# MasterVVK/qwen3-tts-axera-russian

Hardware: AMD Instinct MI355X
Metric: 12Hz codec-tokens/s (codec frames/s, 16 codes each) + RTF, Qwen3-TTS-0.6B (higher is better)
Workload: dtype f16 weights/KV, f32 accumulate (talker+CP); vocoder exact fp32 (f32 MFMA); 1 GPU; configs[2]/[3]: batch=32 mixed ru/en prompts per GPU, 64 frames/utterance/step (prefill + hipGraph decode loop), utterance-sharded DP over 1 GPU(s); batch_per_gpu=32

## Files before the change

### qwen3_tts_axera_russian_amd/csrc/q3_kernels.h

```cpp
#pragma once
#include "q3_common.h"
#include "q3_frag.h"

namespace q3 {

enum { PRO_F16 = 0, PRO_NORM = 1 };
enum { EPI_STORE = 0, EPI_RESID = 1, EPI_SWIGLU = 2 };

struct LinArgs {
    int tl_node = -1;
    const half_t* wp = nullptr;
    int N = 0, K = 0, M = 0;
    int m_begin = 0;
    int swap_grid = 0;
    int nt = 0;
    const half_t* x16 = nullptr;
    const float* ssq = nullptr;
    int ssq_parts = 0;
    float eps = 1e-6f;
    float* y = nullptr;
    int ldy = 0;
    float* h_out = nullptr;
    float* ssq_out = nullptr;
    half_t* xh_out = nullptr;
    const float* gamma = nullptr;
    half_t* act = nullptr;
};
int launch_linear(hipStream_t s, const LinArgs& a, int pro, int epi);
int linear_decode_kbw(int K, int N, int rows);

int launch_pack_linear(hipStream_t s, const half_t* src, int N, int K, half_t* dst, int tile_off,
                       int tile_stride);

enum { ATTN_FUSED = 0, ATTN_PREP = 1, ATTN_ATTEND = 2 };
struct AttnArgs {
    int tl_node = -1;
    float* qkv = nullptr;
// ... 163 lines not shown
    int seen_vocab = 0;
    const float* talker_emb = nullptr;
    int talker_vocab = 0;
    const float* const* cp_tables = nullptr;
    int cp_vocab = 0, n_groups = 15;
    const float* pad_embed = nullptr;
    float* h = nullptr;
    float* ssq = nullptr;
    half_t* xh = nullptr;
    const float* gamma = nullptr;
    int row0 = 0, max_rows = 0, H = 0;
};
int launch_prompt_rows(hipStream_t s, const PromptRowsArgs& a);

int tl_next_node();

int set_linear_tuning(int K, int mt16, int kbw);
int set_linear_split_rows(int on);
int set_linear_narrow8(int on);
int set_linear_wide_tiles(int on);
int set_attn_short(int on);
int set_gemm_min_rows(int n);
int set_gemm_glds(int on);
int reset_linear_knobs();
const char* last_linear_variant();

}
```

### qwen3_tts_axera_russian_amd/csrc/q3_linear.hip

```cpp
#include "q3_kdev.h"

namespace q3 {

__global__ void pack_linear_kernel(const half_t* __restrict__ src, int N, int K, half_t* __restrict__ dst,
                                   int tile_off, int tile_stride) {
    const int KB = K / 32;
    size_t idx = (size_t)blockIdx.x * blockDim.x + threadIdx.x;
    size_t total = (size_t)(N / 16) * KB * 64;
    if (idx >= total) return;
    int lane = (int)(idx & 63);
    size_t blk = idx >> 6;
    int kb = (int)(blk % KB);
    int ts = (int)(blk / KB);
    int n = ts * 16 + (lane & 15);
    int k = kb * 32 + (lane >> 4) * 8;
    h8 v = *(const h8*)(src + (size_t)n * K + k);
    size_t td = (size_t)tile_off + (size_t)ts * tile_stride;
    *(h8*)(dst + ((td * KB + kb) * 64 + lane) * 8) = v;
}

int launch_pack_linear(hipStream_t s, const half_t* src, int N, int K, half_t* dst, int tile_off,
                       int tile_stride) {
    if (N % 16 || K % 32) {
        Q3_LOG("pack_linear: N=%d K=%d not multiples of 16/32", N, K);
// ... 195 lines not shown
    const unsigned nt_ = a.N / (16 * NB16), nr_ = (a.M - a.m_begin + MR - 1) / MR;
    b.swap_grid = nr_ > 2 ? 1 : 0;
    dim3 grid(b.swap_grid ? nr_ : nt_, b.swap_grid ? nt_ : nr_);
    const void* asrc = (const void*)b.x16;
    void* outp = EPI == EPI_STORE ? (void*)b.y : EPI == EPI_RESID ? (void*)b.h_out : (void*)b.act;
    hipLaunchKernelGGL((linear_kernel<NB16, MT16, KBW, NW, PRO, EPI, NT>), grid, dim3(NW * 64), lds, s, b.wp, asrc, b.ssq,
                       b.gamma, outp, b.M, b.N, b.m_begin, b.swap_grid, b.eps, b);
    Q3_HIP(hipGetLastError(), -1);
    return 0;
}

__device__ __forceinline__ void gemm_tile_of_block(int R, int T, int& row_tile, int& col_tile) {
    const int L = blockIdx.x;
    if (T % 8 == 0) {
        const int x = L & 7, j = L >> 3;
        row_tile = j % R;
        col_tile = x + 8 * (j / R);
    } else {
        row_tile = L % R;
        col_tile = L / R;
    }
}

template <int BM, int BN, int PRO, int EPI>
__device__ __forceinline__ void gemm_epilogue(const LinArgs& a, f4 (&acc)[BM / 32][BN / 32], const float* post, int m0,
                                              int tile0, int wm, int wn, int q, int c) {
    constexpr int WM = BM / 32, WN = BN / 32;
#pragma unroll
    for (int i = 0; i < WM; i++) {
#pragma unroll
        for (int r = 0; r < 4; r++) {
            const int mr = (wm * WM + i) * 16 + 4 * q + r;
            const int m = m0 + mr;
            const bool ok = m < a.M;
            const float ps = PRO == PRO_NORM ? post[mr] : 1.0f;
            if (EPI == EPI_SWIGLU) {
#pragma unroll
                for (int j = 0; j < WN; j += 2) {
                    const float g = acc[i][j][r] * ps, u = acc[i][j + 1][r] * ps;
                    const float sg = __fdividef(g, 1.0f + __expf(-g));
                    const int jn = ((tile0 + wn * WN + j) >> 1) * 16 + c;
                    if (ok) a.act[frag_idx(m, jn, a.N / 2)] = sat_half(sg * u);
                }
            } else {
#pragma unroll
                for (int j = 0; j < WN; j++) {
                    const int ng = (tile0 + wn * WN + j) * 16 + c;
                    const float v = acc[i][j][r] * ps;
                    if (EPI == EPI_STORE) {
                        if (ok) a.y[(size_t)m * a.ldy + ng] = v;
                    } else {
                        const size_t hi = frag_idx(m, ng, a.N);
                        const float hn = ok ? a.h_out[hi] + v : 0.f;
                        if (ok) a.h_out[hi] = hn;
                        if (ok && a.xh_out) a.xh_out[hi] = pre_scaled(hn, a.gamma[ng]);
                        const float s2 = group_sum_down<16>(hn * hn);
                        if (ok && c == 0) a.ssq_out[(size_t)m * (a.N / 16) + (ng >> 4)] = s2;
                    }
                }
            }
        }
    }
}

template <int BM, int BN, int KS, int PRO, int EPI>
__global__ void __launch_bounds__(256) gemm_kernel(LinArgs a) {
    constexpr int RA = BM / 16, RB = BN / 16;
    constexpr int NF = (RA + RB) * KS, FPW = NF / 4;
    constexpr int WM = BM / 32, WN = BN / 32;
    static_assert(NF % 4 == 0 && WN % 2 == 0, "tile shape");
    Q3_TL(20 + PRO * 4 + EPI);
    const int tid = threadIdx.x, lane = tid & 63, w = tid >> 6;
    const int wm = w >> 1, wn = w & 1, q = lane >> 4, c = lane & 15;
    int row_tile, col_tile;
    gemm_tile_of_block((a.M - a.m_begin + BM - 1) / BM, a.N / BN, row_tile, col_tile);
    const int m0 = a.m_begin + row_tile * BM;
    const int tile0 = col_tile * RB;
    const int KB = a.K >> 5, NST = KB / KS;
// ... 42 lines not shown
            for (int i = 0; i < FPW; i++) st[i] = *frag_ptr(w * FPW + i, (ks + 1) * KS);
        }
        const h8* cur = lds + (size_t)(ks & 1) * NF * 64;
#pragma unroll
        for (int kk = 0; kk < KS; kk++) {
            h8 af[WM], bf[WN];
#pragma unroll
            for (int i = 0; i < WM; i++) af[i] = cur[((wm * WM + i) * KS + kk) * 64 + lane];
#pragma unroll
            for (int j = 0; j < WN; j++) bf[j] = cur[(RA * KS + (wn * WN + j) * KS + kk) * 64 + lane];
#pragma unroll
            for (int i = 0; i < WM; i++)
#pragma unroll
                for (int j = 0; j < WN; j++)
                    acc[i][j] = __builtin_amdgcn_mfma_f32_16x16x32_f16(af[i], bf[j], acc[i][j], 0, 0, 0);
        }
        if (more) {
            h8* nxt = lds + (size_t)((ks + 1) & 1) * NF * 64;
#pragma unroll
            for (int i = 0; i < FPW; i++) nxt[(w * FPW + i) * 64 + lane] = st[i];
        }
        __syncthreads();
    }
    gemm_epilogue<BM, BN, PRO, EPI>(a, acc, post, m0, tile0, wm, wn, q, c);
}

template <int N>
__device__ __forceinline__ void wait_vmcnt() {
    asm volatile("s_waitcnt vmcnt(%0)" ::"n"(N) : "memory");
}

template <int BM, int BN, int NBUF, int PRO, int EPI, int KS = 2>
__global__ void __launch_bounds__(512) gemm_glds_kernel(LinArgs a) {
    constexpr int RA = BM / 16, RB = BN / 16;
    static_assert(KS % 2 == 0, "two wave groups share a stage's k-blocks");
    constexpr int NF = (RA + RB) * KS, FPW = NF / 8;
    constexpr int WM = BM / 32, WN = BN / 32;
    constexpr int PF = NBUF - 1;
    static_assert(NF % 8 == 0 && WN % 2 == 0, "tile shape");
    static_assert((size_t)NBUF * NF * 1024 >= (size_t)4 * WM * WN * 4 * 64 * 4, "the ring must hold one group's accumulators");
    Q3_TL(24 + PRO * 4 + EPI);
    const int tid = threadIdx.x, lane = tid & 63, w = tid >> 6;
    const int grp = w >> 2, wq = w & 3;
    const int wm = wq >> 1, wn = wq & 1, q = lane >> 4, c = lane & 15;
    int row_tile, col_tile;
    gemm_tile_of_block((a.M - a.m_begin + BM - 1) / BM, a.N / BN, row_tile, col_tile);
    const int m0 = a.m_begin + row_tile * BM;
// ... 25 lines not shown
        for (int r = tid; r < BM; r += 512) {
            const int m = m0 + r;
            float sum = 0.f;
            if (m < a.M) {
                const float4* sp = (const float4*)(a.ssq + (size_t)m * 64);
#pragma unroll
                for (int p = 0; p < 16; p++) {
                    const float4 v = sp[p];
                    sum += (v.x + v.y) + (v.z + v.w);
                }
            }
            post[r] = (1.0f / sqrtf(sum / (float)a.K + a.eps)) * NORM_POST;
        }
    }
    asm volatile("s_waitcnt vmcnt(0)" ::: "memory");
#pragma unroll
    for (int st = 0; st < PF; st++)
        if (st < NST) issue(st);
    f4 acc[WM][WN];
#pragma unroll
    for (int i = 0; i < WM; i++)
#pragma unroll
        for (int j = 0; j < WN; j++) acc[i][j] = (f4){0.f, 0.f, 0.f, 0.f};
    for (int ks = 0; ks < NST; ks++) {
        const int ahead = NST - 1 - ks;
        if (ahead >= PF - 1) wait_vmcnt<(PF - 1) * FPW>();
        else if (PF > 2 && ahead == 1) wait_vmcnt<FPW>();
        else wait_vmcnt<0>();
        __builtin_amdgcn_s_barrier();
        asm volatile("" ::: "memory");
        if (ks + PF < NST) issue(ks + PF);
        const h8* cur = lds + (size_t)(ks % NBUF) * NF * 64;
#pragma unroll
        for (int kk = 0; kk < KS / 2; kk++) {
            const int kb = grp * (KS / 2) + kk;
            h8 af[WM], bf[WN];
#pragma unroll
            for (int i = 0; i < WM; i++) af[i] = cur[((wm * WM + i) * KS + kb) * 64 + lane];
#pragma unroll
            for (int j = 0; j < WN; j++) bf[j] = cur[(RA * KS + (wn * WN + j) * KS + kb) * 64 + lane];
#pragma unroll
            for (int i = 0; i < WM; i++)
#pragma unroll
                for (int j = 0; j < WN; j++)
                    acc[i][j] = __builtin_amdgcn_mfma_f32_16x16x32_f16(af[i], bf[j], acc[i][j], 0, 0, 0);
        }
    }
    __builtin_amdgcn_s_barrier();
    asm volatile("" ::: "memory");
    f4* xch = (f4*)smem;
    if (grp == 1) {
#pragma unroll
        for (int i = 0; i < WM; i++)
#pragma unroll
            for (int j = 0; j < WN; j++) xch[((size_t)wq * WM * WN + i * WN + j) * 64 + lane] = acc[i][j];
    }
    __syncthreads();
    if (grp == 1) return;
#pragma unroll
    for (int i = 0; i < WM; i++)
#pragma unroll
        for (int j = 0; j < WN; j++) {
            const f4 o = xch[((size_t)wq * WM * WN + i * WN + j) * 64 + lane];
            acc[i][j] += o;
        }
    gemm_epilogue<BM, BN, PRO, EPI>(a, acc, post, m0, tile0, wm, wn, q, c);
}

static int g_gemm_glds = env_int("Q3_GEMM_GLDS", 1);
int set_gemm_glds(int on) { g_gemm_glds = on; return 0; }

template <int BM, int BN, int PRO, int EPI>
static int launch_gemm_t(hipStream_t s, const LinArgs& a) {
    LinArgs b = a;
    b.tl_node = tl_next_node();
    dim3 grid(((a.M - a.m_begin + BM - 1) / BM) * (a.N / BN));
    if (g_gemm_glds) {
#ifndef Q3_GEMM_KS_SMALL
#define Q3_GEMM_KS_SMALL 4
#endif
        constexpr int NBUF = (BM + BN) > 256 ? 3 : 4;
        constexpr int KS2 = (BM + BN) <= 128 ? Q3_GEMM_KS_SMALL : 2;
        constexpr size_t lds2 = (size_t)NBUF * ((BM + BN) / 16) * KS2 * 1024 + BM * 4;
        static bool attr2 = false;
        if (!attr2) {
            Q3_HIP(hipFuncSetAttribute((const void*)gemm_glds_kernel<BM, BN, NBUF, PRO, EPI, KS2>,
                                       hipFuncAttributeMaxDynamicSharedMemorySize, (int)lds2), -1);
            attr2 = true;
        }
        if ((a.K >> 5) % KS2) {
            Q3_LOG("launch_gemm: K=%d is no multiple of %d", a.K, 32 * KS2);
            return -1;
        }
        static char name[64];
        if (!name[0])
            snprintf(name, sizeof(name), "gemm_glds<%d,%d,%d,%s,%s,%d>", BM, BN, NBUF, pro_name(PRO), epi_name(EPI), KS2);
        g_last_variant = name;
        hipLaunchKernelGGL((gemm_glds_kernel<BM, BN, NBUF, PRO, EPI, KS2>), grid, dim3(512), lds2, s, b);
    } else if constexpr (BM + BN <= 256) {
        constexpr int KS = 1024 / (BM + BN);
        constexpr size_t lds = (size_t)2 * ((BM + BN) / 16) * KS * 1024;
        static bool attr_set = false;
        if (!attr_set) {
            if (lds > 48 * 1024)
                Q3_HIP(hipFuncSetAttribute((const void*)gemm_kernel<BM, BN, KS, PRO, EPI>,
                                           hipFuncAttributeMaxDynamicSharedMemorySize, (int)lds), -1);
            attr_set = true;
        }
        static char name[64];
        if (!name[0]) snprintf(name, sizeof(name), "gemm<%d,%d,%d,%s,%s>", BM, BN, KS, pro_name(PRO), epi_name(EPI));
        g_last_variant = name;
        hipLaunchKernelGGL((gemm_kernel<BM, BN, KS, PRO, EPI>), grid, dim3(256), lds, s, b);
    } else {
        Q3_LOG("launch_gemm: no register-staged %d x %d tile", BM, BN);
        return -1;
    }
    Q3_HIP(hipGetLastError(), -1);
    return 0;
}
// ... 115 lines not shown
    else
        hipLaunchKernelGGL((linear_narrow_kernel<KBW, NW, false>), dim3(64, groups), dim3(NW * 64), 0, s, a.wp, a.x16, a.h_out, a.gamma,
                           a.ssq_out, a.xh_out, a.M, a.m_begin, node);
    Q3_HIP(hipGetLastError(), -1);
    return 0;
}

#define Q3_LIN_CASE(NB16_, MT16_, KBW_, NW_, PRO_, EPI_)                                   \
    if (nb16 == NB16_ && mt16 == MT16_ && kbw == KBW_ && nw == NW_ && pro == PRO_ && epi == EPI_) \
        return launch_linear_t<NB16_, MT16_, KBW_, NW_, PRO_, EPI_>(s, a);

#define Q3_LIN_MT(NB16_, KBW_, NW_, PRO_, EPI_) \
    Q3_LIN_CASE(NB16_, 1, KBW_, NW_, PRO_, EPI_) \
    Q3_LIN_CASE(NB16_, 2, KBW_, NW_, PRO_, EPI_) \
    Q3_LIN_CASE(NB16_, 4, KBW_, NW_, PRO_, EPI_)

int reset_linear_knobs() {
    memcpy(g_tune_kbw, g_tune_kbw_default, sizeof(g_tune_kbw));
    g_wide_tiles = 0;
    g_split_rows_narrow = 1;
    g_gemm_min_rows = 65;
    g_narrow8 = env_int("Q3_LINEAR_NARROW8", 1);
    g_gemm_glds = env_int("Q3_GEMM_GLDS", 1);
    return 0;
}

static int decode_mt16(int rows, int N) {
    int mt16 = rows <= 16 ? 1 : rows <= 32 ? 2 : 4;
    if (rows > 16 && rows <= 32 && ((g_split_rows_narrow == 1 && N <= 1024) || g_split_rows_narrow == 2)) mt16 = 1;
    return mt16;
}

int linear_decode_kbw(int K, int N, int rows) {
    const int ki = K == 1024 ? 0 : K == 2048 ? 1 : K == 3072 ? 2 : -1;
    if (rows <= 0 || rows >= g_gemm_min_rows || ki < 0 || N % 32) return 0;
    const int mt16 = decode_mt16(rows, N);
    return g_tune_kbw[ki][mt16 == 1 ? 0 : mt16 == 2 ? 1 : 2];
}

int launch_linear(hipStream_t s, const LinArgs& a, int pro, int epi) {
    g_last_variant = "";
    const int rows = a.M - a.m_begin;
    if (rows <= 0) return 0;
    if (rows >= g_gemm_min_rows) return launch_gemm(s, a, pro, epi);
    const int K = a.K;
    int ki = K == 1024 ? 0 : K == 2048 ? 1 : K == 3072 ? 2 : -1;
// ... 32 lines not shown
```

### qwen3_tts_axera_russian_amd/csrc/q3_sample.hip

```cpp
#include "q3_kdev.h"

namespace q3 {

__device__ __forceinline__ void block_argmax(float& v, int& idx, float* sv, int* si) {
    group_argmax_down<64>(v, idx);
    const int w = threadIdx.x >> 6, nw = blockDim.x >> 6;
    if ((threadIdx.x & 63) == 0) {
        sv[w] = v;
        si[w] = idx;
    }
    __syncthreads();
    v = sv[0];
    idx = si[0];
    for (int i = 1; i < nw; i++)
        if (sv[i] > v || (sv[i] == v && si[i] < idx)) {
            v = sv[i];
            idx = si[i];
        }
    __syncthreads();
}

__device__ __forceinline__ float uniform01(unsigned long long seed, unsigned row, unsigned frame, unsigned group) {
    unsigned long long z = seed + 0x9E3779B97F4A7C15ull * (1ull + row + ((unsigned long long)frame << 20) +
                                                            ((unsigned long long)group << 44));
// ... 148 lines not shown
        }
        chosen = pick;
    }
    __syncthreads();
    return chosen;
}

template <class T>
__device__ __forceinline__ T uniform_entry(const T* p, int r) {
    static_assert(sizeof(T) % 4 == 0, "the entry is read as words");
    constexpr int NW = (int)(sizeof(T) / 4);
    const __attribute__((address_space(4))) int* q = (const __attribute__((address_space(4))) int*)(p + r);
    int w[NW];
#pragma unroll
    for (int i = 0; i < NW; i++) w[i] = q[i];
    T e;
    __builtin_memcpy(&e, w, sizeof(e));
    return e;
}
__device__ __forceinline__ SlotParams uniform_slot(const SlotParams* p, int r) { return uniform_entry(p, r); }
__device__ __forceinline__ SlotRules uniform_rules(const SlotRules* p, int r) { return uniform_entry(p, r); }

template <bool SLOTS, bool RULES = false, bool SCORES = false>
__device__ __forceinline__ void talker_sample_row(const TalkerSampleArgs& a) {
    Q3_TL(42);
    __shared__ float sv[16];
    __shared__ int si[16];
    __shared__ float sc_wm[SCORES ? 16 : 1], sc_ws[SCORES ? 16 : 1];
    float sc_m = -INFINITY, sc_s = 0.f;
    __shared__ int win[32];
    __shared__ int nwin;
    const int r = a.row0 + blockIdx.x;
    const int RT = a.R_total > 0 ? a.R_total : a.R;
    const int np = uniform_load(a.n_past + r);
    const int nt = uniform_load(a.n_text + r);
    const bool was_done = uniform_load(a.done + r) != 0;
    float temperature = a.temperature, top_p = a.top_p;
    int top_k = a.top_k, max_frames = a.max_frames;
    int slot_flags = 0;
    if constexpr (SLOTS) {
        const SlotParams sp = uniform_slot(a.slots, r);
        temperature = sp.t_temp;
        top_p = sp.t_top_p;
        top_k = sp.t_top_k;
        max_frames = sp.max_frames;
        slot_flags = sp.flags;
        if (a.text_avail) {
// ... 117 lines not shown
        } else {
            fc[0] = code;
            if constexpr (SCORES) {
                if (a.scores) {
                    const int nw = blockDim.x >> 6;
                    float m = sc_wm[0], sum = 0.f;
                    for (int i = 1; i < nw; i++) m = fmaxf(m, sc_wm[i]);
                    for (int i = 0; i < nw; i++) sum += sc_wm[i] > -INFINITY ? sc_ws[i] * expf(sc_wm[i] - m) : 0.f;
                    float zu = -INFINITY;
                    if (used >= 0 && used < a.V && (used < a.audio_vocab || used == a.eos))
                        zu = nan_as_inf(a.logits[(size_t)r * a.V + used]);
                    a.scores[((size_t)f * RT + r) * 16] = (m < INFINITY && m > -INFINITY) ? zu - m - logf(sum) : __builtin_nanf("");
                }
            }
            a.past[r * 32 + (np & 31)] = used;
            if constexpr (RULES)
                if (a.seen && used >= 0 && used < a.audio_vocab)
                    a.seen[(size_t)r * ((a.audio_vocab + 31) / 32) + (used >> 5)] |= 1u << (used & 31);
            a.n_past[r] = np + 1;
            a.pos[r] = a.pos0[r] + np;
        }
    }
}
__global__ void talker_sample_kernel(TalkerSampleArgs a) { talker_sample_row<false>(a); }
__global__ void talker_sample_kernel_slots(TalkerSampleArgs a) { talker_sample_row<true>(a); }
__global__ void talker_sample_kernel_rules(TalkerSampleArgs a) { talker_sample_row<true, true>(a); }
__global__ void talker_sample_kernel_scores(TalkerSampleArgs a) { talker_sample_row<false, false, true>(a); }
__global__ void talker_sample_kernel_slots_scores(TalkerSampleArgs a) { talker_sample_row<true, false, true>(a); }
__global__ void talker_sample_kernel_rules_scores(TalkerSampleArgs a) { talker_sample_row<true, true, true>(a); }

static size_t sample_lds_bytes_slots(int n) { return (size_t)sample_sort_len(n) * 8; }

static int sample_vocab_refused(const char* who, bool slots, int V, float temperature, int top_k) {
    if (slots && V > SAMPLE_SORT_CAP) {
        Q3_LOG("%s: a vocabulary of %d is beyond the per-slot sampler (sort cap %d)", who, V, SAMPLE_SORT_CAP);
        return -1;
    }
    if (temperature > 1e-6f && effective_top_k(top_k, V) > SAMPLE_SEL_CAP && V > SAMPLE_SORT_CAP) {
        Q3_LOG("%s: top_k=%d over a vocabulary of %d is beyond the device sampler (sort cap %d)", who, top_k, V, SAMPLE_SORT_CAP);
        return -1;
    }
    return 0;
}

int launch_talker_sample(hipStream_t s, const TalkerSampleArgs& a) {
    if (a.R <= 0) return 0;
    if ((a.text_avail && !a.held) || ((a.text_avail || a.held) && !a.slots)) {
        Q3_LOG("talker_sample: text_avail / held need each other and per-slot mode (text_avail %p, held %p, slots %p)",
               (const void*)a.text_avail, (const void*)a.held, (const void*)a.slots);
        return -1;
    }
    if ((a.rules || a.seen) && (!a.slots || (a.rules && !a.seen) || a.audio_vocab <= 0)) {
        Q3_LOG("talker_sample: rules need seen, and both per-slot mode (rules %p, seen %p, slots %p)", (const void*)a.rules,
               (const void*)a.seen, (const void*)a.slots);
        return -1;
    }
    if (sample_vocab_refused("talker_sample", a.slots != nullptr, a.V, a.temperature, a.top_k)) return -1;
    const size_t lds = a.slots ? sample_lds_bytes_slots(a.V) : sample_lds_bytes(a.V, a.top_k, a.temperature);
    TalkerSampleArgs a2 = a;
    a2.tl_node = tl_next_node();
    static void (*const kernels[2][3])(TalkerSampleArgs) = {
        {talker_sample_kernel, talker_sample_kernel_slots, talker_sample_kernel_rules},
        {talker_sample_kernel_scores, talker_sample_kernel_slots_scores, talker_sample_kernel_rules_scores}};
    hipLaunchKernelGGL(kernels[a.scores ? 1 : 0][(a.rules || a.seen) ? 2 : a.slots ? 1 : 0], dim3(a.R), dim3(256), lds, s, a2);
    Q3_HIP(hipGetLastError(), -1);
    return 0;
}

template <bool SLOTS, bool RULES = false, bool SCORES = false>
__device__ __forceinline__ void cp_argmax_row(const CpArgmaxArgs& a) {
    if constexpr (SLOTS)
        Q3_FETCH_ARGS("s"(a.logits), "s"(a.V), "s"(a.H), "s"(a.row0), "s"(a.R_total), "s"(a.R), "s"(a.group), "s"(a.codes), "s"(a.n_frames),
                      "s"(a.frame_cap), "s"(a.next_table), "s"(a.h_out), "s"(a.ssq_out), "s"(a.xh_out), "s"(a.gamma_next),
                      "s"(a.talker_emb), "s"(a.slots), "s"(a.forced), "s"(a.next_qkv), "s"(a.qkv_out), "s"(a.qkv_ld),
                      "s"(a.text_rows), "s"(a.text_avail), "s"(a.text_cap), "s"(a.held));
    else
        Q3_FETCH_ARGS("s"(a.logits), "s"(a.V), "s"(a.H), "s"(a.row0), "s"(a.R_total), "s"(a.R), "s"(a.group), "s"(a.codes), "s"(a.n_frames),
                      "s"(a.frame_cap), "s"(a.next_table), "s"(a.h_out), "s"(a.ssq_out), "s"(a.xh_out), "s"(a.gamma_next),
                      "s"(a.talker_emb), "s"(a.temperature), "s"(a.forced), "s"(a.next_qkv), "s"(a.qkv_out), "s"(a.qkv_ld));
    Q3_TL(43);
    __shared__ float sv[4];
    __shared__ int si[4];
    const int r = a.row0 + blockIdx.x, tid = threadIdx.x;
    const int RT = a.R_total > 0 ? a.R_total : a.R;
    float best = -INFINITY;
    int bidx = 0x7fffffff;
    const float4* lg = (const float4*)(a.logits + (size_t)r * a.V);
// ... 206 lines not shown
```

### qwen3_tts_axera_russian_amd/csrc/q3_test_api.hip

```cpp
#include "q3_enc.h"
#include "q3_model.h"
#include "q3_spk.h"
#include "q3_voc_ops.h"
#include "q3_xlane.h"
#include <chrono>
#include <cstring>
#include <vector>

using namespace q3;

namespace q3 {
template <int OP, int WIDTH>
__global__ void __launch_bounds__(256) xlane_case_kernel(const float* __restrict__ in, int n, float* __restrict__ out_new,
                                                         float* __restrict__ out_shfl) {
    const int i = blockIdx.x * blockDim.x + threadIdx.x;
    const float v = in[i];
    if (OP == 0) {
        out_new[i] = group_sum_down<WIDTH, WIDTH / 2, XlDpp>(v);
        out_shfl[i] = group_sum_down<WIDTH, WIDTH / 2, XlShfl>(v);
    } else if (OP == 1) {
        out_new[i] = group_max_down<WIDTH, WIDTH / 2, XlDpp>(v);
        out_shfl[i] = group_max_down<WIDTH, WIDTH / 2, XlShfl>(v);
    } else {
        float va = v, vb = v;
// ... 22 lines not shown
}
}

namespace {
struct DBuf {
    void* p = nullptr;
    ~DBuf() {
        if (p) hipFree(p);
    }
    bool alloc(size_t n) { return hipMalloc(&p, n ? n : 16) == hipSuccess; }
    bool up(const void* src, size_t n) { return alloc(n) && (n == 0 || hipMemcpy(p, src, n, hipMemcpyHostToDevice) == hipSuccess); }
};
}

extern "C" {

int q3t_set_linear_tuning(int K, int mt16, int kbw) { return set_linear_tuning(K, mt16, kbw); }
int q3t_set_linear_split_rows(int on) { return set_linear_split_rows(on); }
int q3t_set_linear_narrow8(int on) { return set_linear_narrow8(on); }
int q3t_set_linear_wide_tiles(int on) { return set_linear_wide_tiles(on); }
int q3t_set_attn_short(int on) { return set_attn_short(on); }
int q3t_set_gemm_min_rows(int n) { return set_gemm_min_rows(n); }
int q3t_set_gemm_glds(int on) { return set_gemm_glds(on); }
int q3t_reset_linear_knobs() { return reset_linear_knobs(); }
const char* q3t_last_linear_variant() { return last_linear_variant(); }

int q3t_linear(int M, int N, int K, const uint16_t* W, int gateup, int pro, int epi, const uint16_t* x16,
               const float* h, const float* gamma, float eps, float* y_or_h_io, float* ssq_out, uint16_t* act_out,
               int nt) {
    hipStream_t s = nullptr;
    const int Mp = (M + 127) / 128 * 128;
    DBuf dW, dWp, dx, dhrows, dh, dssq, dg, dy, dso, dact, dxh;
    if (!dW.up(W, (size_t)N * K * 2) || !dWp.alloc((size_t)N * K * 2)) return -1;
    if (gateup) {
        if (launch_pack_linear(s, (const half_t*)dW.p, N / 2, K, (half_t*)dWp.p, 0, 2)) return -1;
        if (launch_pack_linear(s, (const half_t*)dW.p + (size_t)(N / 2) * K, N / 2, K, (half_t*)dWp.p, 1, 2)) return -1;
    } else {
        if (launch_pack_linear(s, (const half_t*)dW.p, N, K, (half_t*)dWp.p, 0, 1)) return -1;
    }
    LinArgs a;
    a.wp = (const half_t*)dWp.p;
    a.N = N;
    a.K = K;
    a.M = M;
    a.nt = nt;
    if (pro == PRO_F16) {
// ... 1534 lines not shown
```

### qwen3_tts_axera_russian_amd/hiplib.py

```python
from __future__ import annotations

import ctypes
import os

from . import LIB_PATH, TEST_LIB_PATH

_lib = None
_test_lib = None

c_void_p, c_int, c_float, c_char_p = ctypes.c_void_p, ctypes.c_int, ctypes.c_float, ctypes.c_char_p
f32p = ctypes.POINTER(ctypes.c_float)
i32p = ctypes.POINTER(ctypes.c_int32)
i64p = ctypes.POINTER(ctypes.c_int64)
u16p = ctypes.POINTER(ctypes.c_uint16)
i16p = ctypes.POINTER(ctypes.c_int16)


class SlotParamsC(ctypes.Structure):
    _fields_ = [("max_frames", ctypes.c_int32), ("temperature", ctypes.c_float), ("top_k", ctypes.c_int32),
                ("top_p", ctypes.c_float), ("cp_temperature", ctypes.c_float), ("cp_top_k", ctypes.c_int32),
                ("seed", ctypes.c_uint64), ("utt", ctypes.c_int32), ("reserved", ctypes.c_int32)]


class KernelSlotParamsC(ctypes.Structure):
# ... 235 lines not shown
    _sig(lib, "q3t_talker_score_case", c_int, talker_case + [i32p, i32p, c_void_p, u32p, f32p])
    _sig(lib, "q3t_cp_score_case", c_int, cp_case + [f32p, i32p, c_int, i32p, c_void_p, f32p])
    _sig(lib, "q3t_prompt_rows_seen_case", c_int, [i32p, c_int, i32p, i32p, f32p, c_int, f32p, c_int, c_int, c_int, f32p, c_int,
                                                   c_int, c_int, c_int, c_int, f32p, f32p, f32p, u16p, c_int, u32p, c_int])
    _sig(lib, "q3t_final_norm_case", c_int, [f32p, f32p, c_int, c_int, c_int, f32p, c_float, c_int, c_int, i32p, c_int, c_int,
                                             c_int, c_int, c_int, f32p, f32p, u16p, f32p, f32p, u16p])
    _sig(lib, "q3t_gather_embed_case", c_int, [f32p, c_int, c_int, i32p, c_int, i32p, c_int, c_int, i32p, c_int, c_int, c_int,
                                               f32p, f32p, f32p, u16p])
    _sig(lib, "q3t_feedback_case", c_int, [i32p, c_int, f32p, c_int, f32p, c_int, c_int, f32p, c_int, f32p, f32p, f32p, u16p])
    _sig(lib, "q3t_prompt_rows_case", c_int, [i32p, c_int, i32p, i32p, f32p, c_int, f32p, c_int, c_int, c_int, f32p, c_int,
                                              c_int, c_int, c_int, c_int, f32p, f32p, f32p, u16p, c_int])
    _sig(lib, "q3t_prefix_move_case", c_int, [u16p, u16p, c_int, c_int, c_int, c_int, u16p, c_int, c_int, f32p, f32p, f32p,
                                              c_int, c_int, c_int, i32p])
    _sig(lib, "q3t_attn", c_int, [c_int, c_int, c_int, f32p, f32p, f32p, c_float, f32p, f32p, c_int, i32p, i32p, c_int,
                                  c_int, c_int, c_int, u16p, u16p, c_int, c_int, i32p, c_int, c_int, c_int, c_int, u16p])
    _sig(lib, "q3t_voc_attn", c_int, [c_int, f32p, f32p, c_int, c_int, c_int, c_int, c_int, c_float])
    _sig(lib, "q3t_xlane_case", c_int, [c_int, c_int, c_int, f32p, f32p, f32p])
    _sig(lib, "q3t_set_linear_split_rows", c_int, [c_int])
    _sig(lib, "q3t_set_linear_narrow8", c_int, [c_int])
    _sig(lib, "q3t_set_linear_wide_tiles", c_int, [c_int])
    _sig(lib, "q3t_set_attn_short", c_int, [c_int])
    _sig(lib, "q3t_set_gemm_min_rows", c_int, [c_int])
    _sig(lib, "q3t_set_gemm_glds", c_int, [c_int])
    _sig(lib, "q3t_inspect_weights", c_int, [ctypes.c_char_p, ctypes.c_char_p, ctypes.c_char_p, c_int])
    _sig(lib, "q3t_bench_linear", c_float, [c_int, c_int, c_int, c_int, c_int, c_int, c_int, c_int])
    _sig(lib, "q3t_bench_chain", c_float, [c_int, c_int, c_int, c_int, c_int, c_int])
    _sig(lib, "q3t_cp_model_load", c_void_p, [c_char_p])
    _sig(lib, "q3t_cp_model_free", None, [c_void_p])
    _sig(lib, "q3t_cp_qkv_ld", c_int, [c_void_p])
    _sig(lib, "q3t_cp_qkv_serves", c_int, [c_void_p, c_int])
    _sig(lib, "q3t_cp_qkv_tab", c_int, [c_void_p, c_int, i32p, c_int, f32p])
    _sig(lib, "q3t_cp_qkv_live", c_int, [c_void_p, c_int, i32p, c_int, c_int, f32p])
    _sig(lib, "q3t_enc_stream_embeddings", c_int, [c_void_p, c_int, i32p, f32p, i32p, i32p, i64p, ctypes.c_int64, i64p, f32p, i32p])
    i64s = ctypes.POINTER(ctypes.c_longlong)
    _sig(lib, "q3t_enc_stream_plan", c_int, [i32p, i32p, c_int, ctypes.c_longlong, ctypes.c_longlong, c_int, i64s, i64s, i64s])
    _sig(lib, "q3t_enc_rvq_tile", c_int, [c_int])
    _sig(lib, "q3t_enc_rvq_case", c_int, [f32p, c_int, c_int, c_int, c_int, c_int, c_int, c_int, f32p, i64p])
    _sig(lib, "q3t_enc_conv_in_case", c_int, [f32p, c_int, c_int, f32p, f32p, c_int, c_int, f32p, c_int, i32p, f32p])
    u8p = ctypes.POINTER(ctypes.c_uint8)
    _sig(lib, "q3t_dequant_case", c_int, [c_int, u8p, ctypes.c_longlong, c_int, c_int, c_int, c_int, u16p, f32p, i32p])
    _sig(lib, "q3t_spk_mel", c_int, [c_void_p, f32p, i32p, c_int, f32p, i32p, i32p])
    _sig(lib, "q3t_spk_stage", c_int, [c_void_p, f32p, i32p, c_int, c_int, f32p, i32p, i32p])
    _sig(lib, "q3t_spk_unfold_case", c_int, [f32p, c_int, c_int, f32p, c_int, c_int, i32p, c_int, c_int, c_int, c_int, f32p])
    _sig(lib, "q3t_spk_place_case", c_int, [f32p, c_int, c_int, c_int, c_int, c_int, c_int, c_int, c_int, f32p])
    _sig(lib, "q3t_spk_rowmean_case", c_int, [f32p, c_int, i32p, c_int, f32p])
    _sig(lib, "q3t_spk_rowstat_case", c_int, [f32p, c_int, i32p, c_int, f32p])
# ... 19 lines not shown
```

Measured before the change: 10530 codec_frames/s.

## Prefetch residual rows in GEMM epilogue and register-cache talker sampler logits

Two independent changes, both on by default. The split-K GEMM with a residual epilogue now loads the residual h and gamma values into registers during the last K stage, so those global loads overlap the final MFMA work instead of stalling the epilogue. The talker sampler kernel is rewritten to load each logits row into registers with float4 reads and to build a shared-memory bitmap of the repetition window, replacing per-element window scans. The old sampler is kept behind an env toggle, and the new code raises register pressure and relies on the bitmap being large enough for the vocabulary.

```diff
diff --git a/qwen3_tts_axera_russian_amd/csrc/q3_kernels.h b/qwen3_tts_axera_russian_amd/csrc/q3_kernels.h
--- a/qwen3_tts_axera_russian_amd/csrc/q3_kernels.h
+++ b/qwen3_tts_axera_russian_amd/csrc/q3_kernels.h
@@ -13,6 +13,7 @@
     int N = 0, K = 0, M = 0;
     int m_begin = 0;
     int swap_grid = 0;
+    int gemm_opts = 0;
     int nt = 0;
     const half_t* x16 = nullptr;
     const float* ssq = nullptr;
@@ -222,6 +223,9 @@
 int set_attn_short(int on);
 int set_gemm_min_rows(int n);
 int set_gemm_glds(int on);
+enum { GEMM_OPT_EARLY_RESID = 2 };
+int set_gemm_opts(int mask);
+int set_talker_sample_serial(int on);
 int reset_linear_knobs();
 const char* last_linear_variant();
 
diff --git a/qwen3_tts_axera_russian_amd/csrc/q3_linear.hip b/qwen3_tts_axera_russian_amd/csrc/q3_linear.hip
--- a/qwen3_tts_axera_russian_amd/csrc/q3_linear.hip
+++ b/qwen3_tts_axera_russian_amd/csrc/q3_linear.hip
@@ -241,9 +241,33 @@
     }
 }
 
+template <int BM, int BN>
+struct ResidPre {
+    float h[BM / 32][4][BN / 32];
+    float g[BN / 32];
+};
+template <int BM, int BN>
+__device__ __forceinline__ void gemm_resid_prefetch(const LinArgs& a, ResidPre<BM, BN>& p, int m0, int tile0, int wm, int wn,
+                                                    int q, int c) {
+    constexpr int WM = BM / 32, WN = BN / 32;
+#pragma unroll
+    for (int j = 0; j < WN; j++) {
+        const int ng = (tile0 + wn * WN + j) * 16 + c;
+        p.g[j] = a.xh_out ? a.gamma[ng] : 0.f;
+#pragma unroll
+        for (int i = 0; i < WM; i++)
+#pragma unroll
+            for (int r = 0; r < 4; r++) {
+                const int m = m0 + (wm * WM + i) * 16 + 4 * q + r;
+                p.h[i][r][j] = m < a.M ? a.h_out[frag_idx(m, ng, a.N)] : 0.f;
+            }
+    }
+}
+
 template <int BM, int BN, int PRO, int EPI>
 __device__ __forceinline__ void gemm_epilogue(const LinArgs& a, f4 (&acc)[BM / 32][BN / 32], const float* post, int m0,
-                                              int tile0, int wm, int wn, int q, int c) {
+                                              int tile0, int wm, int wn, int q, int c, const ResidPre<BM, BN>& pre,
+                                              bool use_pre) {
     constexpr int WM = BM / 32, WN = BN / 32;
 #pragma unroll
     for (int i = 0; i < WM; i++) {
@@ -270,9 +294,9 @@
                         if (ok) a.y[(size_t)m * a.ldy + ng] = v;
                     } else {
                         const size_t hi = frag_idx(m, ng, a.N);
-                        const float hn = ok ? a.h_out[hi] + v : 0.f;
+                        const float hn = ok ? (use_pre ? pre.h[i][r][j] : a.h_out[hi]) + v : 0.f;
                         if (ok) a.h_out[hi] = hn;
-                        if (ok && a.xh_out) a.xh_out[hi] = pre_scaled(hn, a.gamma[ng]);
+                        if (ok && a.xh_out) a.xh_out[hi] = pre_scaled(hn, use_pre ? pre.g[j] : a.gamma[ng]);
                         const float s2 = group_sum_down<16>(hn * hn);
                         if (ok && c == 0) a.ssq_out[(size_t)m * (a.N / 16) + (ng >> 4)] = s2;
                     }
@@ -361,7 +385,7 @@
         }
         __syncthreads();
     }
-    gemm_epilogue<BM, BN, PRO, EPI>(a, acc, post, m0, tile0, wm, wn, q, c);
+    gemm_epilogue<BM, BN, PRO, EPI>(a, acc, post, m0, tile0, wm, wn, q, c, ResidPre<BM, BN>{}, false);
 }
 
 template <int N>
@@ -433,6 +457,9 @@
     for (int i = 0; i < WM; i++)
 #pragma unroll
         for (int j = 0; j < WN; j++) acc[i][j] = (f4){0.f, 0.f, 0.f, 0.f};
+    constexpr bool CAN_EARLY = EPI == EPI_RESID && BM + BN <= 128;
+    ResidPre<CAN_EARLY ? BM : 32, CAN_EARLY ? BN : 32> rpre = {};
+    const bool early = CAN_EARLY && grp == 0 && (a.gemm_opts & GEMM_OPT_EARLY_RESID);
     for (int ks = 0; ks < NST; ks++) {
         const int ahead = NST - 1 - ks;
         if (ahead >= PF - 1) wait_vmcnt<(PF - 1) * FPW>();
@@ -441,6 +468,8 @@
         __builtin_amdgcn_s_barrier();
         asm volatile("" ::: "memory");
         if (ks + PF < NST) issue(ks + PF);
+        if constexpr (CAN_EARLY)
+            if (early && ks == NST - 1) gemm_resid_prefetch<BM, BN>(a, rpre, m0, tile0, wm, wn, q, c);
         const h8* cur = lds + (size_t)(ks % NBUF) * NF * 64;
 #pragma unroll
         for (int kk = 0; kk < KS / 2; kk++) {
@@ -475,11 +504,15 @@
             const f4 o = xch[((size_t)wq * WM * WN + i * WN + j) * 64 + lane];
             acc[i][j] += o;
         }
-    gemm_epilogue<BM, BN, PRO, EPI>(a, acc, post, m0, tile0, wm, wn, q, c);
+    if constexpr (CAN_EARLY) gemm_epilogue<BM, BN, PRO, EPI>(a, acc, post, m0, tile0, wm, wn, q, c, rpre, early);
+    else gemm_epilogue<BM, BN, PRO, EPI>(a, acc, post, m0, tile0, wm, wn, q, c, ResidPre<BM, BN>{}, false);
 }
 
 static int g_gemm_glds = env_int("Q3_GEMM_GLDS", 1);
 int set_gemm_glds(int on) { g_gemm_glds = on; return 0; }
+constexpr int GEMM_OPTS_DEFAULT = GEMM_OPT_EARLY_RESID;
+static int g_gemm_opts = env_int("Q3_GEMM_OPTS", GEMM_OPTS_DEFAULT);
+int set_gemm_opts(int mask) { g_gemm_opts = mask < 0 ? env_int("Q3_GEMM_OPTS", GEMM_OPTS_DEFAULT) : mask; return 0; }
 
 template <int BM, int BN, int PRO, int EPI>
 static int launch_gemm_t(hipStream_t s, const LinArgs& a) {
@@ -503,9 +536,12 @@
             Q3_LOG("launch_gemm: K=%d is no multiple of %d", a.K, 32 * KS2);
             return -1;
         }
-        static char name[64];
+        if (BM + BN <= 128 && EPI == EPI_RESID) b.gemm_opts = g_gemm_opts & GEMM_OPT_EARLY_RESID;
+        static char names[2][64];
+        char* name = names[b.gemm_opts ? 1 : 0];
         if (!name[0])
-            snprintf(name, sizeof(name), "gemm_glds<%d,%d,%d,%s,%s,%d>", BM, BN, NBUF, pro_name(PRO), epi_name(EPI), KS2);
+            snprintf(name, 64, "gemm_glds<%d,%d,%d,%s,%s,%d>%s", BM, BN, NBUF, pro_name(PRO), epi_name(EPI), KS2,
+                     (BM + BN <= 128 && EPI == EPI_RESID && !b.gemm_opts) ? "/late" : "");
         g_last_variant = name;
         hipLaunchKernelGGL((gemm_glds_kernel<BM, BN, NBUF, PRO, EPI, KS2>), grid, dim3(512), lds2, s, b);
     } else if constexpr (BM + BN <= 256) {
@@ -667,6 +703,7 @@
     g_gemm_min_rows = 65;
     g_narrow8 = env_int("Q3_LINEAR_NARROW8", 1);
     g_gemm_glds = env_int("Q3_GEMM_GLDS", 1);
+    g_gemm_opts = env_int("Q3_GEMM_OPTS", GEMM_OPTS_DEFAULT);
     return 0;
 }
 
diff --git a/qwen3_tts_axera_russian_amd/csrc/q3_sample.hip b/qwen3_tts_axera_russian_amd/csrc/q3_sample.hip
--- a/qwen3_tts_axera_russian_amd/csrc/q3_sample.hip
+++ b/qwen3_tts_axera_russian_amd/csrc/q3_sample.hip
@@ -194,7 +194,7 @@
 __device__ __forceinline__ SlotRules uniform_rules(const SlotRules* p, int r) { return uniform_entry(p, r); }
 
 template <bool SLOTS, bool RULES = false, bool SCORES = false>
-__device__ __forceinline__ void talker_sample_row(const TalkerSampleArgs& a) {
+__device__ __forceinline__ void talker_sample_row_serial(const TalkerSampleArgs& a) {
     Q3_TL(42);
     __shared__ float sv[16];
     __shared__ int si[16];
@@ -358,12 +358,238 @@
         }
     }
 }
-__global__ void talker_sample_kernel(TalkerSampleArgs a) { talker_sample_row<false>(a); }
-__global__ void talker_sample_kernel_slots(TalkerSampleArgs a) { talker_sample_row<true>(a); }
-__global__ void talker_sample_kernel_rules(TalkerSampleArgs a) { talker_sample_row<true, true>(a); }
-__global__ void talker_sample_kernel_scores(TalkerSampleArgs a) { talker_sample_row<false, false, true>(a); }
-__global__ void talker_sample_kernel_slots_scores(TalkerSampleArgs a) { talker_sample_row<true, false, true>(a); }
-__global__ void talker_sample_kernel_rules_scores(TalkerSampleArgs a) { talker_sample_row<true, true, true>(a); }
+constexpr int SAMPLE_REG = 12;
+constexpr int SAMPLE_MAP_BITS = 4096;
+constexpr int SAMPLE_THREADS = 256;
+template <bool SLOTS, bool RULES = false, bool SCORES = false>
+__device__ __forceinline__ void talker_sample_row(const TalkerSampleArgs& a) {
+    Q3_FETCH_ARGS("s"(a.logits), "s"(a.V), "s"(a.row0), "s"(a.R_total), "s"(a.R), "s"(a.audio_vocab), "s"(a.eos), "s"(a.past),
+                  "s"(a.n_past), "s"(a.n_text), "s"(a.done), "s"(a.codes), "s"(a.n_frames), "s"(a.frame_cap), "s"(a.pos0),
+                  "s"(a.pos), "s"(a.forced), "s"(a.slots), "s"(a.text_avail));
+    Q3_TL(42);
+    __shared__ float sv[16];
+    __shared__ int si[16];
+    __shared__ float sc_wm[SCORES ? 16 : 1], sc_ws[SCORES ? 16 : 1];
+    float sc_m = -INFINITY, sc_s = 0.f;
+    __shared__ int win[32];
+    __shared__ unsigned rep_map[SAMPLE_MAP_BITS / 32];
+    const int tid = threadIdx.x;
+    constexpr int nthr = SAMPLE_THREADS;
+    const int r = a.row0 + blockIdx.x;
+    const int RT = a.R_total > 0 ? a.R_total : a.R;
+    const int V = a.V;
+    const float* row = a.logits + (size_t)r * V;
+    const bool vec = !SCORES && (V & 3) == 0 && ((size_t)a.logits & 15) == 0;
+    float e[SAMPLE_REG];
+    if (vec) {
+#pragma unroll
+        for (int j = 0; j < SAMPLE_REG / 4; j++) {
+            const int i4 = tid + nthr * j;
+            float4 t = make_float4(0.f, 0.f, 0.f, 0.f);
+            if (i4 * 4 < V) t = ((const float4*)row)[i4];
+            e[4 * j] = t.x;
+            e[4 * j + 1] = t.y;
+            e[4 * j + 2] = t.z;
+            e[4 * j + 3] = t.w;
+        }
+    } else {
+#pragma unroll
+        for (int k = 0; k < SAMPLE_REG; k++) {
+            const int v = tid + nthr * k;
+            e[k] = v < V ? row[v] : 0.f;
+        }
+    }
+    const int ring_id = tid < 32 ? a.past[r * 32 + tid] : 0;
+    const int np = uniform_load(a.n_past + r);
+    const int nt = uniform_load(a.n_text + r);
+    const bool was_done = uniform_load(a.done + r) != 0;
+    const int f = uniform_load(a.n_frames + r);
+    const int pos0 = uniform_load(a.pos0 + r);
+    int fz = -1;
+    if (a.forced && f >= 0 && f < a.frame_cap) fz = uniform_load(a.forced + ((size_t)f * RT + r) * 16);
+    asm volatile("" ::: "memory");
+    for (int i = tid; i < SAMPLE_MAP_BITS / 32; i += nthr) rep_map[i] = 0u;
+    float temperature = a.temperature, top_p = a.top_p;
+    int top_k = a.top_k, max_frames = a.max_frames;
+    int slot_flags = 0;
+    SlotParams sp;
+    if constexpr (SLOTS) {
+        sp = uniform_slot(a.slots, r);
+        temperature = sp.t_temp;
+        top_p = sp.t_top_p;
+        top_k = sp.t_top_k;
+        max_frames = sp.max_frames;
+        slot_flags = sp.flags;
+        if (a.text_avail) {
+            const int avail = uniform_load(a.text_avail + r);
+            const int gen = np - sp.prompt;
+            const bool held = (slot_flags & 3) == 3 && !was_done && gen >= 1 && gen >= avail && np < max_frames;
+            if (tid == 0) a.held[r] = held ? 1 : 0;
+            if (held) return;
+        }
+    }
+    float rep_penalty = a.rep_penalty;
+    int rep_window = 30;
+    double eos_boost = 15.0, eos_force = 2.0;
+    bool add_boost = true, may_force = true, eos_early = false;
+    const unsigned* seen_row = nullptr;
+    if constexpr (RULES) {
+        if (a.rules) {
+            const SlotRules ru = uniform_rules(a.rules, r);
+            rep_penalty = ru.rep_penalty;
+            rep_window = ru.rep_window < 0 ? 0 : ru.rep_window > 30 ? 30 : ru.rep_window;
+            eos_boost = (double)ru.eos_boost;
+            eos_force = (double)ru.eos_force;
+            add_boost = ru.eos_boost != 0.f;
+            may_force = ru.eos_force != 0.f;
+            eos_early = np < ru.min_past;
+            if (rep_window == 0) seen_row = a.seen + (size_t)r * ((a.audio_vocab + 31) / 32);
+        }
+    }
+    const int nw_ = np < rep_window ? np : rep_window;
+    double progress = 0.0;
+    float boost = 0.f;
+    bool force_eos = false;
+    if (nt > 0) {
+        const double expected = (double)nt * 3.0;
+        progress = (double)np / expected;
+        if (progress > 0.8) {
+            double b = (progress - 0.8) / 0.7;
+            if (b > 1.0) b = 1.0;
+            boost = (float)(b * eos_boost);
+        }
+        if (may_force && progress > eos_force) force_eos = true;
+    }
+    const bool eos_masked = a.ignore_eos || (SLOTS && (slot_flags & 2)) || (RULES && eos_early);
+    __syncthreads();
+    if (tid < 32) {
+        const int age = (np - 1 - tid) & 31;
+        if (age < nw_) {
+            win[age] = ring_id;
+            if ((unsigned)ring_id < (unsigned)SAMPLE_MAP_BITS) atomicOr(&rep_map[ring_id >> 5], 1u << (ring_id & 31));
+        }
+    }
+    __syncthreads();
+    float best = -INFINITY;
+    int bidx = 0x7fffffff;
+    extern __shared__ float slg[];
+    __shared__ float selv[64];
+    __shared__ int seli[64];
+    const bool stochastic = temperature > 1e-6f;
+    auto consider = [&](int v, float raw, bool rep) {
+        float l = nan_as_inf(raw);
+        if constexpr (SCORES) {
+            if ((v < a.audio_vocab || v == a.eos) && l > -INFINITY) {
+                if (l > sc_m) {
+                    sc_s = sc_s * expf(sc_m - l) + 1.f;
+                    sc_m = l;
+                } else {
+                    sc_s += expf(l - sc_m);
+                }
+            }
+        }
+        if (v >= a.audio_vocab && v != a.eos) l = -1e10f;
+        if (v == a.eos) {
+            if (eos_masked) l = -1e10f;
+            else if (nt > 0 && progress > 0.8 && add_boost) l += boost;
+        }
+        if constexpr (RULES)
+            if (seen_row && v < a.audio_vocab) rep = (seen_row[v >> 5] >> (v & 31)) & 1u;
+        if (rep) l = l > 0.f ? __fdiv_rn(l, rep_penalty) : l * rep_penalty;
+        if (stochastic) slg[v] = l;
+        if (l > best || (l == best && v < bidx)) {
+            best = l;
+            bidx = v;
+        }
+    };
+    static_assert(SAMPLE_REG * SAMPLE_THREADS <= SAMPLE_MAP_BITS, "an entry held in a register has a bit in the map");
+    auto ent = [&](int k) { return vec ? (tid + nthr * (k >> 2)) * 4 + (k & 3) : tid + nthr * k; };
+    unsigned mw[SAMPLE_REG];
+#pragma unroll
+    for (int k = 0; k < SAMPLE_REG; k++) {
+        const int v = ent(k);
+        mw[k] = rep_map[(v < V ? v : 0) >> 5];
+    }
+#pragma unroll
+    for (int k = 0; k < SAMPLE_REG; k++) {
+        const int v = ent(k);
+        if (v < V) consider(v, e[k], (mw[k] >> (v & 31)) & 1u);
+    }
+    for (int v = nthr * SAMPLE_REG + tid; v < V; v += nthr) {
+        bool rep = false;
+        if (v < SAMPLE_MAP_BITS) rep = (rep_map[v >> 5] >> (v & 31)) & 1u;
+        else
+            for (int i = 0; i < nw_; i++) rep |= (win[i] == v);
+        consider(v, row[v], rep);
+    }
+    if constexpr (SCORES) {
+        const float wm = wave_max(sc_m);
+        const float ws = wave_sum(sc_m > -INFINITY ? sc_s * expf(sc_m - wm) : 0.f);
+        if ((tid & 63) == 0) {
+            sc_wm[tid >> 6] = wm;
+            sc_ws[tid >> 6] = ws;
+        }
+    }
+    if (stochastic) {
+        __syncthreads();
+        float u;
+        if constexpr (SLOTS) {
+            u = uniform01(sp.seed, sp.no_row ? 0u : (unsigned)r, (unsigned)f, 0u);
+        } else {
+            u = uniform01(a.seed_ptr ? a.seed_ptr[r] : a.seed, (unsigned)r, (unsigned)f, 0u);
+        }
+        bidx = block_sample_topk(slg, V, top_k, temperature, top_p, u, sv, si, selv, seli);
+    } else {
+        block_argmax(best, bidx, sv, si);
+        if (bidx >= V) bidx = a.eos;
+    }
+    if (tid == 0) {
+        int code = bidx;
+        if (force_eos && !eos_masked) code = a.eos;
+        bool fin = was_done || code == a.eos || code >= a.audio_vocab || (max_frames > 0 && np >= max_frames);
+        if (!SLOTS || !fin || f <= a.frame_cap) a.n_frames[r] = f + 1;
+        const bool keep = f < a.frame_cap;
+        int* fc = a.codes + ((size_t)(keep ? f : 0) * RT + r) * 16;
+        int used = code;
+        if (a.forced && keep && !fin && fz >= 0) used = fz;
+        if (fin || !keep) {
+            a.done[r] = 1;
+            if (keep) fc[0] = -1;
+        } else {
+            fc[0] = code;
+            if constexpr (SCORES) {
+                if (a.scores) {
+                    const int nw = nthr >> 6;
+                    float m = sc_wm[0], sum = 0.f;
+                    for (int i = 1; i < nw; i++) m = fmaxf(m, sc_wm[i]);
+                    for (int i = 0; i < nw; i++) sum += sc_wm[i] > -INFINITY ? sc_ws[i] * expf(sc_wm[i] - m) : 0.f;
+                    float zu = -INFINITY;
+                    if (used >= 0 && used < V && (used < a.audio_vocab || used == a.eos))
+                        zu = nan_as_inf(a.logits[(size_t)r * V + used]);
+                    a.scores[((size_t)f * RT + r) * 16] = (m < INFINITY && m > -INFINITY) ? zu - m - logf(sum) : __builtin_nanf("");
+                }
+            }
+            a.past[r * 32 + (np & 31)] = used;
+            if constexpr (RULES)
+                if (a.seen && used >= 0 && used < a.audio_vocab)
+                    a.seen[(size_t)r * ((a.audio_vocab + 31) / 32) + (used >> 5)] |= 1u << (used & 31);
+            a.n_past[r] = np + 1;
+            a.pos[r] = pos0 + np;
+        }
+    }
+}
+__global__ void __launch_bounds__(SAMPLE_THREADS) talker_sample_kernel(TalkerSampleArgs a) { talker_sample_row<false>(a); }
+__global__ void __launch_bounds__(SAMPLE_THREADS) talker_sample_kernel_slots(TalkerSampleArgs a) { talker_sample_row<true>(a); }
+__global__ void __launch_bounds__(SAMPLE_THREADS) talker_sample_kernel_rules(TalkerSampleArgs a) { talker_sample_row<true, true>(a); }
+__global__ void __launch_bounds__(SAMPLE_THREADS) talker_sample_kernel_scores(TalkerSampleArgs a) { talker_sample_row<false, false, true>(a); }
+__global__ void __launch_bounds__(SAMPLE_THREADS) talker_sample_kernel_slots_scores(TalkerSampleArgs a) { talker_sample_row<true, false, true>(a); }
+__global__ void __launch_bounds__(SAMPLE_THREADS) talker_sample_kernel_rules_scores(TalkerSampleArgs a) { talker_sample_row<true, true, true>(a); }
+__global__ void talker_sample_serial_kernel(TalkerSampleArgs a) { talker_sample_row_serial<false>(a); }
+__global__ void talker_sample_serial_kernel_slots(TalkerSampleArgs a) { talker_sample_row_serial<true>(a); }
+__global__ void talker_sample_serial_kernel_rules(TalkerSampleArgs a) { talker_sample_row_serial<true, true>(a); }
+__global__ void talker_sample_serial_kernel_scores(TalkerSampleArgs a) { talker_sample_row_serial<false, false, true>(a); }
+__global__ void talker_sample_serial_kernel_slots_scores(TalkerSampleArgs a) { talker_sample_row_serial<true, false, true>(a); }
+__global__ void talker_sample_serial_kernel_rules_scores(TalkerSampleArgs a) { talker_sample_row_serial<true, true, true>(a); }
 
 static size_t sample_lds_bytes_slots(int n) { return (size_t)sample_sort_len(n) * 8; }
 
@@ -376,6 +602,12 @@
         Q3_LOG("%s: top_k=%d over a vocabulary of %d is beyond the device sampler (sort cap %d)", who, top_k, V, SAMPLE_SORT_CAP);
         return -1;
     }
+    return 0;
+}
+
+static int g_sample_serial = getenv("Q3_SAMPLE_SERIAL") ? atoi(getenv("Q3_SAMPLE_SERIAL")) : 0;
+int set_talker_sample_serial(int on) {
+    g_sample_serial = on < 0 ? (getenv("Q3_SAMPLE_SERIAL") ? atoi(getenv("Q3_SAMPLE_SERIAL")) : 0) : on;
     return 0;
 }
 
@@ -395,10 +627,13 @@
     const size_t lds = a.slots ? sample_lds_bytes_slots(a.V) : sample_lds_bytes(a.V, a.top_k, a.temperature);
     TalkerSampleArgs a2 = a;
     a2.tl_node = tl_next_node();
-    static void (*const kernels[2][3])(TalkerSampleArgs) = {
-        {talker_sample_kernel, talker_sample_kernel_slots, talker_sample_kernel_rules},
-        {talker_sample_kernel_scores, talker_sample_kernel_slots_scores, talker_sample_kernel_rules_scores}};
-    hipLaunchKernelGGL(kernels[a.scores ? 1 : 0][(a.rules || a.seen) ? 2 : a.slots ? 1 : 0], dim3(a.R), dim3(256), lds, s, a2);
+    static void (*const kernels[2][2][3])(TalkerSampleArgs) = {
+        {{talker_sample_kernel, talker_sample_kernel_slots, talker_sample_kernel_rules},
+         {talker_sample_kernel_scores, talker_sample_kernel_slots_scores, talker_sample_kernel_rules_scores}},
+        {{talker_sample_serial_kernel, talker_sample_serial_kernel_slots, talker_sample_serial_kernel_rules},
+         {talker_sample_serial_kernel_scores, talker_sample_serial_kernel_slots_scores, talker_sample_serial_kernel_rules_scores}}};
+    hipLaunchKernelGGL(kernels[g_sample_serial ? 1 : 0][a.scores ? 1 : 0][(a.rules || a.seen) ? 2 : a.slots ? 1 : 0], dim3(a.R),
+                       dim3(SAMPLE_THREADS), lds, s, a2);
     Q3_HIP(hipGetLastError(), -1);
     return 0;
 }
diff --git a/qwen3_tts_axera_russian_amd/csrc/q3_test_api.hip b/qwen3_tts_axera_russian_amd/csrc/q3_test_api.hip
--- a/qwen3_tts_axera_russian_amd/csrc/q3_test_api.hip
+++ b/qwen3_tts_axera_russian_amd/csrc/q3_test_api.hip
@@ -68,6 +68,8 @@
 int q3t_set_attn_short(int on) { return set_attn_short(on); }
 int q3t_set_gemm_min_rows(int n) { return set_gemm_min_rows(n); }
 int q3t_set_gemm_glds(int on) { return set_gemm_glds(on); }
+int q3t_set_gemm_opts(int mask) { return set_gemm_opts(mask); }
+int q3t_set_talker_sample_serial(int on) { return set_talker_sample_serial(on); }
 int q3t_reset_linear_knobs() { return reset_linear_knobs(); }
 const char* q3t_last_linear_variant() { return last_linear_variant(); }
 
diff --git a/qwen3_tts_axera_russian_amd/hiplib.py b/qwen3_tts_axera_russian_amd/hiplib.py
--- a/qwen3_tts_axera_russian_amd/hiplib.py
+++ b/qwen3_tts_axera_russian_amd/hiplib.py
@@ -281,6 +281,8 @@
     _sig(lib, "q3t_set_attn_short", c_int, [c_int])
     _sig(lib, "q3t_set_gemm_min_rows", c_int, [c_int])
     _sig(lib, "q3t_set_gemm_glds", c_int, [c_int])
+    _sig(lib, "q3t_set_talker_sample_serial", c_int, [c_int])
+    _sig(lib, "q3t_set_gemm_opts", c_int, [c_int])
     _sig(lib, "q3t_inspect_weights", c_int, [ctypes.c_char_p, ctypes.c_char_p, ctypes.c_char_p, c_int])
     _sig(lib, "q3t_bench_linear", c_float, [c_int, c_int, c_int, c_int, c_int, c_int, c_int, c_int])
     _sig(lib, "q3t_bench_chain", c_float, [c_int, c_int, c_int, c_int, c_int, c_int])
```

Result: no change. 10560 codec_frames/s (median of 6 runs) (+0.3%).
